# marthinwurer/gcmiipy

Hardware: AMD Instinct MI355X
Metric: cell-updates/s (C-grid Matsuno step) (higher is better)
Workload: dtype f64; 1 GPU; 2-D shallow water + theta + viscosity + van-Leer tracer, 4096x2048 fp64 (BASELINE configs[2]); variant=fused, decomposition=1 latitude band(s)

## Files before the change

### gcmiipy_amd/csrc/gcm_math.h

```cpp
#pragma once
#include <hip/hip_runtime.h>

#include "sw2d_kernels.h"

namespace gcm {

constexpr double kG = 9.8;
constexpr double kRd = 287.0;
constexpr double kRv = 461.0;
constexpr double kCp = 1004.0;
constexpr double kKappa = 287.0 / 1004.0;
constexpr double kP0 = 100000.0;
constexpr double kMuAir = 18.5 * 1e-6;

__device__ __forceinline__ double rcp(double x) {
    double r = __builtin_amdgcn_rcp(x);
    double e = __builtin_fma(-x, r, 1.0);
    r = __builtin_fma(r, e, r);
    e = __builtin_fma(-x, r, 1.0);
    r = __builtin_fma(r, e, r);
    return r;
}
__device__ __forceinline__ float rcp(float x) { return __builtin_amdgcn_rcpf(x); }
constexpr double kTinyF64 = 2.2250738585072014e-308;

constexpr double kBinom1 = kKappa;
constexpr double kBinom2 = kBinom1 * (kKappa - 1) / 2;
constexpr double kBinom3 = kBinom2 * (kKappa - 2) / 3;
constexpr double kBinom4 = kBinom3 * (kKappa - 3) / 4;
constexpr double kBinom5 = kBinom4 * (kKappa - 4) / 5;
constexpr double kBinom6 = kBinom5 * (kKappa - 5) / 6;
constexpr double kBinom7 = kBinom6 * (kKappa - 6) / 7;

__host__ __device__ __forceinline__ double exner(double p, const double *tab ) {
#if defined(__HIP_DEVICE_COMPILE__)
    const int hi = __double2hiint(p);
    const int e = ((hi >> 20) & 0x7ff) - 1023;
    const int idx = (hi >> 14) & 63;
    const double m = __hiloint2double((hi & 0x000fffff) | 0x3ff00000, __double2loint(p));
    const int ec = min(max(e, -64), 63);
#else
    unsigned long long bits;
    __builtin_memcpy(&bits, &p, sizeof bits);
    const int hi = (int)(unsigned)(bits >> 32);
    const int e = ((hi >> 20) & 0x7ff) - 1023;
    const int idx = (hi >> 14) & 63;
    const unsigned long long mbits = ((unsigned long long)(unsigned)((hi & 0x000fffff) | 0x3ff00000) << 32) | (bits & 0xffffffffull);
    double m;
    __builtin_memcpy(&m, &mbits, sizeof m);
    const int ec = e < -64 ? -64 : (e > 63 ? 63 : e);
#endif
    const double E = tab[ec + 64];
    const double rc = tab[128 + 2 * idx], ck = tab[129 + 2 * idx];
    const double t = __builtin_fma(m, rc, -1.0);
    const double t2 = t * t, t4 = t2 * t2;
    const double q12 = __builtin_fma(t, kBinom2, kBinom1);
    const double q34 = __builtin_fma(t, kBinom4, kBinom3);
    const double q56 = __builtin_fma(t, kBinom6, kBinom5);
    const double hi3 = __builtin_fma(t4, kBinom7, __builtin_fma(t2, q56, q34));
    const double poly = __builtin_fma(t * t2, hi3, __builtin_fma(t, q12, 1.0));
    const double r = E * ck * poly;
    const bool ok = (hi >= 0) && (e >= -64) && (e <= 63);
    return ok ? r : __builtin_nan("");
}
__device__ __forceinline__ float exner(float p, const double *tab) { return (float)exner((double)p, tab); }

__device__ __forceinline__ double from_west(double x) {
    int lo = __double2loint(x), hi = __double2hiint(x);
    lo = __builtin_amdgcn_update_dpp(0, lo, 0x138 , 0xf, 0xf, true);
    hi = __builtin_amdgcn_update_dpp(0, hi, 0x138, 0xf, 0xf, true);
    return __hiloint2double(hi, lo);
}
__device__ __forceinline__ double from_east(double x) {
    int lo = __double2loint(x), hi = __double2hiint(x);
    lo = __builtin_amdgcn_update_dpp(0, lo, 0x130 , 0xf, 0xf, true);
    hi = __builtin_amdgcn_update_dpp(0, hi, 0x130, 0xf, 0xf, true);
    return __hiloint2double(hi, lo);
}
__device__ __forceinline__ float from_west(float x) {
    return __int_as_float(__builtin_amdgcn_update_dpp(0, __float_as_int(x), 0x138 , 0xf, 0xf, true));
}
__device__ __forceinline__ float from_east(float x) {
    return __int_as_float(__builtin_amdgcn_update_dpp(0, __float_as_int(x), 0x130 , 0xf, 0xf, true));
}
typedef float f32x2 __attribute__((ext_vector_type(2)));
__device__ __forceinline__ f32x2 rcp(f32x2 x) { return f32x2{rcp(x.x), rcp(x.y)}; }
__device__ __forceinline__ f32x2 exner(f32x2 p, const double *tab) { return f32x2{exner(p.x, tab), exner(p.y, tab)}; }
__device__ __forceinline__ f32x2 from_west(f32x2 x) { return f32x2{from_west(x.y), x.x}; }
__device__ __forceinline__ f32x2 from_east(f32x2 x) { return f32x2{x.y, from_east(x.x)}; }
__device__ __forceinline__ int sign_word(double x) { return __double2hiint(x); }
__device__ __forceinline__ int sign_word(float x) { return __float_as_int(x); }


template <typename T>
__device__ __forceinline__ T adv_vel_u(T uc, T uw, T ue, T un, T us, T vc, T vw, T vs, T vsw, T h_dx) {
    T u_ipj = ue + uc, u_imj = uw + uc, v_ijm = vw + vc, v_ijp = vsw + vs;
    T du_ipj = ue - uc, du_imj = uc - uw, du_ijp = us - uc, du_ijm = uc - un;
    return (u_ipj * du_ipj + u_imj * du_imj + v_ijp * du_ijp + v_ijm * du_ijm) * h_dx;
}

template <typename T>
__device__ __forceinline__ T adv_vel_v(T vc, T vw, T ve, T vn, T vs, T uc, T un, T uw, T usw, T h_dx) {
    T v_ijp = vs + vc, v_ijm = vn + vc, u_ipj = uc + un, u_imj = uw + usw;
    T dv_ipj = ve - vc, dv_imj = vc - vw, dv_ijp = vs - vc, dv_ijm = vc - vn;
    return (u_ipj * dv_ipj + u_imj * dv_imj + v_ijp * dv_ijp + v_ijm * dv_ijm) * h_dx;
}

template <typename T>
__device__ __forceinline__ T geo_grad(T p_next, T pc, T g_dx) {
    return (p_next - pc) * g_dx;
}

template <typename T>
__device__ __forceinline__ T adv_geo(T uc, T uw, T vc, T vn, T pc, T pw, T pe, T pn, T ps, T h_dx) {
    T up_imj = (pw + pc) * uw;
    T up_ipj = (pe + pc) * uc;
    T vp_ijm = (pn + pc) * vn;
    T vp_ijp = (ps + pc) * vc;
    return (up_ipj - up_imj) * h_dx + (vp_ijp - vp_ijm) * h_dx;
}

template <typename T>
__device__ __forceinline__ T visc_u(T uc, T uw, T ue, T un, T us, T mu_dx2) {
    T top = us + un + ue + uw - T(4.0) * uc;
    return top * mu_dx2;
}

template <typename T>
struct Thermo { T t_over_p, geo, st; };
template <typename T>
__device__ __forceinline__ Thermo<T> thermo(T p, T t, const double *tab, T rcp_p) {
    T temp = t * exner(p, tab);
    Thermo<T> r;
    r.t_over_p = temp * rcp_p;
    r.geo = temp * T(kRd / kG);
    r.st = p * t;
    return r;
}
template <typename T>
__device__ __forceinline__ Thermo<T> thermo(T p, T t, const double *tab) {
    return thermo(p, t, tab, rcp(p));
}

template <bool LIMIT, typename T>
__device__ __forceinline__ T face_flux(T vel, T qm1, T q0, T q1, T q2, T dtdx) {
    const bool pos = vel > T(0.0);
    const T vd = vel * dtdx;
    const T f_low = (pos ? q0 : q1) * vd;
    if (!LIMIT) return f_low;
    const T f_high = vd * ((q0 + q1) * T(0.5));
    const T b = q1 - q0;
    const T num = pos ? q0 - qm1 : q2 - q1;
    const T an = fabs(num), ab = fabs(b);
    const bool same = (sign_word(num) ^ sign_word(b)) >= 0;
    T phi;
    if constexpr (sizeof(T) == 8) {
        phi = same && an >= kTinyF64 && ab >= kTinyF64 ? (an + an) * rcp(ab + an) : T(0.0);
    } else {
        phi = same && an > T(0.0) && ab > T(0.0) ? fmin((an + an) * rcp(ab + an), T(2.0)) : T(0.0);
    }
    return f_low + phi * (f_high - f_low);
}
template <bool LIMIT>
__device__ __forceinline__ f32x2 face_flux(f32x2 vel, f32x2 qm1, f32x2 q0, f32x2 q1, f32x2 q2, f32x2 dtdx) {
    return f32x2{face_flux<LIMIT>(vel.x, qm1.x, q0.x, q1.x, q2.x, dtdx.x),
                 face_flux<LIMIT>(vel.y, qm1.y, q0.y, q1.y, q2.y, dtdx.y)};
}

}
```

### gcmiipy_amd/csrc/sw2d_impl.h

```cpp
#pragma once
#include <hip/hip_runtime.h>

#include <cstdlib>
#include <type_traits>

#include "gcm_math.h"
#include "sw2d_kernels.h"

namespace gcm {

__device__ __forceinline__ long row_off(int j, int H, int W, bool wrap) {
    if (wrap) {
        j %= H;
        if (j < 0) j += H;
    }
    return (long)j * W;
}

template <typename T>
__device__ __forceinline__ Sw2dArgsT<T> member_args(const Sw2dArgsT<T> &a0, int m) {
    Sw2dArgsT<T> a = a0;
    const long o = (long)m * a0.mstride;
    auto mv = [o](auto *p) { return p ? p + o : p; };
    a.bu = mv(a.bu); a.bv = mv(a.bv); a.bp = mv(a.bp); a.bt = mv(a.bt); a.bq = mv(a.bq);
    a.su = mv(a.su); a.sv = mv(a.sv); a.sp = mv(a.sp); a.st = mv(a.st);
    a.sgeo = mv(a.sgeo); a.sirho = mv(a.sirho); a.sst = mv(a.sst);
    a.ou = mv(a.ou); a.ov = mv(a.ov); a.op = mv(a.op); a.ot = mv(a.ot); a.oq = mv(a.oq);
    a.dgeo = mv(a.dgeo); a.dirho = mv(a.dirho); a.dst = mv(a.dst);
    return a;
}

template <typename T>
__global__ __launch_bounds__(256) void sw2d_derive_kernel(Sw2dArgsT<T> a0) {
    const Sw2dArgsT<T> a = member_args(a0, blockIdx.z);
    __shared__ double tab[kExnerTabDoubles];
    tab[threadIdx.y * 64 + threadIdx.x] = a.exner_tab[threadIdx.y * 64 + threadIdx.x];
    __syncthreads();
    const int i = blockIdx.x * 64 + threadIdx.x;
    const int j = a.j0 + blockIdx.y * 4 + threadIdx.y;
    if (i >= a.W || j >= a.j1) return;
    const long o = (long)j * a.W + i;
    Thermo<T> th = thermo(a.sp[o], a.st[o], tab);
    a.dgeo[o] = th.geo;
    a.dirho[o] = th.t_over_p;
    a.dst[o] = th.st;
}

template <typename T, bool TEMP>
__global__ __launch_bounds__(256) void sw2d_stage_kernel(Sw2dArgsT<T> a0) {
    const Sw2dArgsT<T> a = member_args(a0, blockIdx.z);
    const int W = a.W, H = a.H;
    const int i = blockIdx.x * 64 + threadIdx.x;
    const int j = a.j0 + blockIdx.y * 4 + threadIdx.y;
    if (i >= W || j >= a.j1) return;
    const bool wrap = a.wrap_j;
    const int iw = i == 0 ? W - 1 : i - 1, ie = i == W - 1 ? 0 : i + 1;
    const long rc = row_off(j, H, W, wrap), rn = row_off(j - 1, H, W, wrap),
               rs = row_off(j + 1, H, W, wrap);
    const T uc = a.su[rc + i], uw = a.su[rc + iw], ue = a.su[rc + ie], un = a.su[rn + i], us = a.su[rs + i],
            usw = a.su[rs + iw];
    const T vc = a.sv[rc + i], vw = a.sv[rc + iw], ve = a.sv[rc + ie], vn = a.sv[rn + i], vs = a.sv[rs + i],
            vsw = a.sv[rs + iw];
    const T pc = a.sp[rc + i], pw = a.sp[rc + iw], pe = a.sp[rc + ie], pn = a.sp[rn + i], ps = a.sp[rs + i];
    T gc = pc, ge = pe, gs = ps;
    if (TEMP) {
        gc = a.sgeo[rc + i];
        ge = a.sgeo[rc + ie];
        gs = a.sgeo[rs + i];
    }
    T du = adv_vel_u(uc, uw, ue, un, us, vc, vw, vs, vsw, a.h_dx) + geo_grad(ge, gc, a.g_dx);
    T dv = adv_vel_v(vc, vw, ve, vn, vs, uc, un, uw, usw, a.h_dx) + geo_grad(gs, gc, a.g_dx);
    if (TEMP) {
        const T vis = visc_u(uc, uw, ue, un, us, a.mu_dx2) * a.sirho[rc + i];
        du -= vis;
        dv -= vis;
    }
    const T dp = adv_geo(uc, uw, vc, vn, pc, pw, pe, pn, ps, a.h_dx);
    const long o = (long)j * W + i;
    const T bp = a.bp[o];
    const T pnew = bp - a.dt * dp;
    a.ou[o] = a.bu[o] - a.dt * du;
    a.ov[o] = a.bv[o] - a.dt * dv;
    a.op[o] = pnew;
    if (TEMP) {
        const T dst = adv_geo(uc, uw, vc, vn, a.sst[rc + i], a.sst[rc + iw], a.sst[rc + ie],
                                   a.sst[rn + i], a.sst[rs + i], a.h_dx);
        const T tt = bp * a.bt[o] - a.dt * dst;
        a.ot[o] = tt * rcp(pnew);
    }
}

template <typename T, int AXIS, bool LIMIT>
__global__ __launch_bounds__(256) void tracer_axis_kernel(Sw2dArgsT<T> a0, const T *qin, T *qout) {
    const Sw2dArgsT<T> a = member_args(a0, blockIdx.z);
    qin += blockIdx.z * a0.mstride;
    qout += blockIdx.z * a0.mstride;
    const int W = a.W, H = a.H;
    const int i = blockIdx.x * 64 + threadIdx.x;
    const int j = a.j0 + blockIdx.y * 4 + threadIdx.y;
    if (i >= W || j >= a.j1) return;
    const bool wrap = a.wrap_j;
    T f, fm;
    const long rc = row_off(j, H, W, wrap);
    if (AXIS == 0) {
        const long r1 = row_off(j + 1, H, W, wrap), r2 = row_off(j + 2, H, W, wrap),
                   rm = row_off(j - 1, H, W, wrap), rmm = row_off(j - 2, H, W, wrap);
        const T qmm = qin[rmm + i], qm = qin[rm + i], q0 = qin[rc + i], q1 = qin[r1 + i], q2 = qin[r2 + i];
        f = face_flux<LIMIT>(a.bv[rc + i], qm, q0, q1, q2, a.dtdx);
        fm = face_flux<LIMIT>(a.bv[rm + i], qmm, qm, q0, q1, a.dtdx);
        qout[(long)j * W + i] = q0 - f + fm;
    } else {
        auto wi = [W](int x) { x %= W; return x < 0 ? x + W : x; };
        const int i1 = wi(i + 1), i2 = wi(i + 2), im = wi(i - 1), imm = wi(i - 2);
        const T qmm = qin[rc + imm], qm = qin[rc + im], q0 = qin[rc + i], q1 = qin[rc + i1], q2 = qin[rc + i2];
        f = face_flux<LIMIT>(a.bu[rc + i], qm, q0, q1, q2, a.dtdx);
        fm = face_flux<LIMIT>(a.bu[rc + im], qmm, qm, q0, q1, a.dtdx);
        qout[(long)j * W + i] = q0 - f + fm;
    }
}

template <typename T>
static dim3 cell_grid(const Sw2dArgsT<T> &a) {
    return dim3((a.W + 63) / 64, (a.j1 - a.j0 + 3) / 4, a.members);
}

template <typename T>
void launch_sw2d_derive(const Sw2dArgsT<T> &a, hipStream_t s) {
    if (a.j1 <= a.j0) return;
    hipLaunchKernelGGL(sw2d_derive_kernel<T>, cell_grid(a), dim3(64, 4), 0, s, a);
}

template <typename T>
void launch_sw2d_stage(const Sw2dArgsT<T> &a, bool temp, hipStream_t s) {
    if (a.j1 <= a.j0) return;
    if (temp)
        hipLaunchKernelGGL((sw2d_stage_kernel<T, true>), cell_grid(a), dim3(64, 4), 0, s, a);
    else
        hipLaunchKernelGGL((sw2d_stage_kernel<T, false>), cell_grid(a), dim3(64, 4), 0, s, a);
}

template <typename T>
void launch_tracer_axis(const Sw2dArgsT<T> &a, int axis, bool limit, const T *q_in, T *q_out, hipStream_t s) {
    if (a.j1 <= a.j0) return;
    dim3 g = cell_grid(a), b(64, 4);
    if (axis == 0) {
        if (limit) hipLaunchKernelGGL((tracer_axis_kernel<T, 0, true>), g, b, 0, s, a, q_in, q_out);
        else hipLaunchKernelGGL((tracer_axis_kernel<T, 0, false>), g, b, 0, s, a, q_in, q_out);
    } else {
        if (limit) hipLaunchKernelGGL((tracer_axis_kernel<T, 1, true>), g, b, 0, s, a, q_in, q_out);
        else hipLaunchKernelGGL((tracer_axis_kernel<T, 1, false>), g, b, 0, s, a, q_in, q_out);
    }
}

template <typename T>
struct Row {
    T u, uw, v, vw, p, st, g, irho;
};

template <bool TEMP, typename T>
__device__ __forceinline__ void make_row_r(Row<T> &r, T u, T v, T p, T t, const double *tab, T rcp_p) {
    r.u = u;
    r.v = v;
    r.p = p;
    r.uw = from_west(u);
    r.vw = from_west(v);
    if (TEMP) {
        Thermo<T> th = thermo(p, t, tab, rcp_p);
        r.st = th.st;
        r.g = th.geo;
        r.irho = th.t_over_p;
    } else {
        r.st = T(0.0);
        r.g = p;
        r.irho = T(0.0);
    }
}

template <bool TEMP, typename T>
__device__ __forceinline__ void make_row(Row<T> &r, T u, T v, T p, T t, const double *tab) {
    make_row_r<TEMP>(r, u, v, p, t, tab, TEMP ? rcp(p) : T(0.0));
}

template <typename T>
struct Tend {
    T du, dv, dp, dst;
};

template <bool TEMP, typename T>
__device__ __forceinline__ Tend<T> tendencies(const Row<T> &RM, const Row<T> &R0, const Row<T> &RP, T g_dx, T h_dx,
                                              T mu_dx2) {
    const T ue = from_east(R0.u), ve = from_east(R0.v);
    const T uw = R0.uw, vw = R0.vw, usw = RP.uw, vsw = RP.vw;
    const T pw = from_west(R0.p), pe = from_east(R0.p);
    const T ge = TEMP ? from_east(R0.g) : pe;
    Tend<T> t;
    t.du = adv_vel_u(R0.u, uw, ue, RM.u, RP.u, R0.v, vw, RP.v, vsw, h_dx) +
           geo_grad(ge, R0.g, g_dx);
    t.dv = adv_vel_v(R0.v, vw, ve, RM.v, RP.v, R0.u, RM.u, uw, usw, h_dx) +
           geo_grad(RP.g, R0.g, g_dx);
    if (TEMP) {
        const T vis = visc_u(R0.u, uw, ue, RM.u, RP.u, mu_dx2) * R0.irho;
        t.du -= vis;
        t.dv -= vis;
    }
    t.dp = adv_geo(R0.u, uw, R0.v, RM.v, R0.p, pw, pe, RM.p, RP.p, h_dx);
    t.dst = T(0.0);
    if (TEMP) {
        const T stw = from_west(R0.st), ste = from_east(R0.st);
        t.dst = adv_geo(R0.u, uw, R0.v, RM.v, R0.st, stw, ste, RM.st, RP.st, h_dx);
    }
    return t;
}

template <typename T>
struct Raw {
    T u, v, p, t, q;
};

constexpr unsigned kNoStore = 0x80000000u;
__device__ __forceinline__ void store_row_lanes(double *row, int W, unsigned lane_off, double x) {
    typedef unsigned int u32x2 __attribute__((ext_vector_type(2)));
    const __amdgpu_buffer_rsrc_t rs = __builtin_amdgcn_make_buffer_rsrc(row, 0, W * 8, 0x00020000);
    __builtin_amdgcn_raw_buffer_store_b64(__builtin_bit_cast(u32x2, x), rs, (int)lane_off, 0, 0);
}

__device__ __forceinline__ double own_copy(double x) {
    double y;
    asm volatile("v_mov_b64 %0, %1" : "=v"(y) : "v"(x) : "memory");
    return y;
}

template <typename T, bool TEMP, int TRACER, bool WRAPJ, bool STREAM = false, int CPL = 1>
struct FusedCtx {
    using Real = std::conditional_t<CPL == 2, f32x2, T>;
    using V = Real;
    const Sw2dArgsT<T> &a;
    const double *tab;
    int ci, col, ja, jb;
    bool store_lane;
    V f0_prev;

    __device__ __forceinline__ Raw<V> load(int j) const {
        const long o = row_off(j, a.H, a.W, WRAPJ) + ci;
        Raw<V> r;
        if constexpr (CPL == 2) {
            auto ld = [o](const T *p) {
                const f32x2 *q = (const f32x2 *)(p + o);
                return STREAM ? __builtin_nontemporal_load(q) : *q;
            };
            r.u = ld(a.bu);
            r.v = ld(a.bv);
            r.p = ld(a.bp);
            r.t = TEMP ? ld(a.bt) : V(0.0f);
            r.q = TRACER ? ld(a.bq) : V(0.0f);
        } else if (STREAM) {
            r.u = __builtin_nontemporal_load(&a.bu[o]);
            r.v = __builtin_nontemporal_load(&a.bv[o]);
            r.p = __builtin_nontemporal_load(&a.bp[o]);
            r.t = TEMP ? __builtin_nontemporal_load(&a.bt[o]) : T(0.0);
            r.q = TRACER ? __builtin_nontemporal_load(&a.bq[o]) : T(0.0);
        } else {
            r.u = a.bu[o];
            r.v = a.bv[o];
            r.p = a.bp[o];
            r.t = TEMP ? a.bt[o] : T(0.0);
            r.q = TRACER ? a.bq[o] : T(0.0);
        }
        return r;
    }

    template <bool FETCH = true, int AHEAD = 3, int LEAD = -1, bool ROWBUF = false>
    __device__ __forceinline__ void iter(int r, Row<V> &BM, Row<V> &B0, Row<V> &BP, Row<V> &SN, Row<V> &SM,
                                         Row<V> &S0, Raw<V> &nxt, V &qmm, V &qm, V &q0, V &qp) {
        const V dt = V(a.dt), g_dx = V(a.g_dx), h_dx = V(a.h_dx), mu_dx2 = V(a.mu_dx2), dtdx = V(a.dtdx);
        {
            const Tend<V> t = tendencies<TEMP>(BM, B0, BP, g_dx, h_dx, mu_dx2);
            const V us = B0.u - dt * t.du;
            const V vs = B0.v - dt * t.dv;
            const V ps = B0.p - dt * t.dp;
            V ts = V(0.0), rps = V(0.0);
            if (TEMP) {
                rps = rcp(ps);
                ts = (B0.st - dt * t.dst) * rps;
            }
            make_row_r<TEMP>(SN, us, vs, ps, ts, tab, rps);
        }
        V f0_cur = V(0.0);
        if (TRACER && (LEAD < 0 ? r >= ja : LEAD >= 1)) f0_cur = face_flux<TRACER == 2>(BM.v, qmm, qm, q0, qp, dtdx);
        if (LEAD < 0 ? r >= ja + 1 : LEAD >= 2) {
            const Tend<V> t = tendencies<TEMP>(SM, S0, SN, g_dx, h_dx, mu_dx2);
            const V un = BM.u - dt * t.du;
            const V vn = BM.v - dt * t.dv;
            const V pn = BM.p - dt * t.dp;
            V tn = V(0.0), qn = V(0.0);
            if (TEMP) tn = (BM.st - dt * t.dst) * rcp(pn);
            if (TRACER) {
                const V qs = qm - f0_cur + f0_prev;
                const V qs_w = from_west(qs), qs_e = from_east(qs);
                const V qs_ee = from_east(qs_e);
                const V f1 = face_flux<TRACER == 2>(BM.u, qs_w, qs, qs_e, qs_ee, dtdx);
                qn = qs - f1 + from_west(f1);
            }
            if constexpr (ROWBUF) {
                const long o = (long)(r - 1) * a.W;
                const unsigned lane_off = store_lane ? (unsigned)col * 8u : kNoStore;
                store_row_lanes(a.ou + o, a.W, lane_off, un);
                store_row_lanes(a.ov + o, a.W, lane_off, vn);
                store_row_lanes(a.op + o, a.W, lane_off, pn);
                if (TEMP) store_row_lanes(a.ot + o, a.W, lane_off, tn);
                if (TRACER) store_row_lanes(a.oq + o, a.W, lane_off, qn);
            } else if (store_lane) {
                const long o = (long)(r - 1) * a.W + col;
                if constexpr (CPL == 2) {
                    auto st = [o](T *p, V x) { *(V *)(p + o) = x; };
                    st(a.ou, un);
                    st(a.ov, vn);
                    st(a.op, pn);
                    if (TEMP) st(a.ot, tn);
                    if (TRACER) st(a.oq, qn);
                } else {
                    a.ou[o] = un;
                    a.ov[o] = vn;
                    a.op[o] = pn;
                    if (TEMP) a.ot[o] = tn;
                    if (TRACER) a.oq[o] = qn;
                }
            }
        }
        f0_prev = f0_cur;
        if constexpr (AHEAD == 3) {
            make_row<TEMP>(BM, nxt.u, nxt.v, nxt.p, nxt.t, tab);
        } else {
            make_row<TEMP>(BM, own_copy(nxt.u), own_copy(nxt.v), own_copy(nxt.p), TEMP ? own_copy(nxt.t) : nxt.t, tab);
        }
        if (TRACER) {
            qmm = qm;
            qm = q0;
            q0 = qp;
            if constexpr (AHEAD == 3) qp = nxt.q;
            else qp = own_copy(nxt.q);
        }
        if constexpr (AHEAD == 3) {
            if (FETCH && r + 3 <= jb + 1) nxt = load(r + 3);
        } else {
            nxt = load(min(r + AHEAD, jb + 1));
        }
    }
};

template <int N, int PRE, class Ctx, typename T = typename Ctx::Real>
__device__ __forceinline__ void preloaded_iters(Ctx &c, const Raw<T> (&pre)[PRE + 4], Row<T> &A, Row<T> &B, Row<T> &C,
                                                Row<T> &X, Row<T> &Y, Row<T> &Z, Raw<T> &nxt, T &qmm, T &qm, T &q0,
                                                T &qp) {
    if constexpr (N < PRE + 2) {
        const int r = c.ja - 1 + N;
        if (r > c.jb) return;
        c.template iter<false>(r, A, B, C, X, Y, Z, nxt, qmm, qm, q0, qp);
        if constexpr (N < PRE) nxt = pre[N + 4];
        preloaded_iters<N + 1, PRE>(c, pre, B, C, A, Y, Z, X, nxt, qmm, qm, q0, qp);
    }
}

template <typename T, bool TEMP, int TRACER, bool WRAPJ, int PRE = 0, bool STREAM = false, int CPL = 1, int DEPTH = 1>
__global__ __launch_bounds__(64, DEPTH == 3 ? 2 : (CPL == 2 && TRACER != 0) ? 3 : 1) void sw2d_fused_kernel(Sw2dArgsT<T> a0) {
    using Ctx = FusedCtx<T, TEMP, TRACER, WRAPJ, STREAM, CPL>;
    using V = typename Ctx::Real;
    constexpr int kCols = sw2d_fused_strip_cols(CPL);
    const int W = a0.W;
    const int lane = threadIdx.x;
    const int strips = (W + kCols - 1) / kCols;
    const int per_xcd = gridDim.x / 8;
    int tile = (blockIdx.x % 8) * per_xcd + blockIdx.x / 8;
    int member = 0;
    if (a0.members > 1) {
        const int per_member = strips * ((a0.j1 - a0.j0 + a0.rows_per_band - 1) / a0.rows_per_band);
        member = tile / per_member;
        if (member >= a0.members) return;
        tile -= member * per_member;
    }
    const int band = tile / strips;
    const int i0 = (tile - band * strips) * kCols;
    const Sw2dArgsT<T> a = member_args(a0, member);
    __shared__ double tab[kExnerTabDoubles];
    if (TEMP) {
        for (int k = 0; k < kExnerTabDoubles / 64; ++k) tab[lane + 64 * k] = a.exner_tab[lane + 64 * k];
        __syncthreads();
    }
    Ctx c{a, tab};
    c.ja = a.j0 + band * a.rows_per_band;
    c.jb = min(c.ja + a.rows_per_band, a.j1);
    if (c.ja >= c.jb) return;
    c.col = i0 - 2 * CPL + CPL * lane;
    c.ci = c.col % W;
    if (c.ci < 0) c.ci += W;
    c.store_lane = lane >= 2 && lane < 62 && c.col < W;
    c.f0_prev = V(0.0);
    const int ja = c.ja, jb = c.jb;

    Row<V> A, B, C, X, Y, Z;
    if constexpr (PRE > 0) {
        Raw<V> pre[PRE + 4];
#pragma unroll
        for (int n = 0; n < PRE + 4; ++n) pre[n] = c.load(min(ja - 2 + n, jb + 1));
        make_row<TEMP>(A, pre[0].u, pre[0].v, pre[0].p, pre[0].t, tab);
        make_row<TEMP>(B, pre[1].u, pre[1].v, pre[1].p, pre[1].t, tab);
        make_row<TEMP>(C, pre[2].u, pre[2].v, pre[2].p, pre[2].t, tab);
        V qmm = V(0.0), qm = pre[0].q, q0 = pre[1].q, qp = pre[2].q;
        Raw<V> nxt = pre[3];
        X = Y = Z = A;
        preloaded_iters<0, PRE>(c, pre, A, B, C, X, Y, Z, nxt, qmm, qm, q0, qp);
        return;
    }
    if constexpr (DEPTH == 3) {
        static_assert(PRE == 0 && CPL == 1, "the deep march is the rolling form with one column per lane");
        const Raw<V> w0 = c.load(ja - 2), w1 = c.load(ja - 1), w2 = c.load(ja);
        Raw<V> n0 = c.load(ja + 1), n1 = c.load(ja + 2), n2 = c.load(min(ja + 3, jb + 1));
        make_row<TEMP>(A, w0.u, w0.v, w0.p, w0.t, tab);
        make_row<TEMP>(B, w1.u, w1.v, w1.p, w1.t, tab);
        make_row<TEMP>(C, w2.u, w2.v, w2.p, w2.t, tab);
        V qmm = V(0.0), qm = w0.q, q0 = w1.q, qp = w2.q;
        X = Y = Z = A;
        c.template iter<true, 5, 0, true>(ja - 1, A, B, C, X, Y, Z, n0, qmm, qm, q0, qp);
        c.template iter<true, 5, 1, true>(ja, B, C, A, Y, Z, X, n1, qmm, qm, q0, qp);
        int r = ja + 1;
        for (; r + 2 <= jb; r += 3) {
            c.template iter<true, 5, 2, true>(r, C, A, B, Z, X, Y, n2, qmm, qm, q0, qp);
            c.template iter<true, 5, 2, true>(r + 1, A, B, C, X, Y, Z, n0, qmm, qm, q0, qp);
            c.template iter<true, 5, 2, true>(r + 2, B, C, A, Y, Z, X, n1, qmm, qm, q0, qp);
        }
        if (r <= jb) {
            c.template iter<false, 3, 2, true>(r, C, A, B, Z, X, Y, n2, qmm, qm, q0, qp);
            if (r + 1 <= jb) c.template iter<false, 3, 2, true>(r + 1, A, B, C, X, Y, Z, n0, qmm, qm, q0, qp);
        }
        return;
    }
    Raw<V> x = c.load(ja - 2);
    make_row<TEMP>(A, x.u, x.v, x.p, x.t, tab);
    V qmm = V(0.0), qm = x.q;
    x = c.load(ja - 1);
    make_row<TEMP>(B, x.u, x.v, x.p, x.t, tab);
    V q0 = x.q;
    x = c.load(ja);
    make_row<TEMP>(C, x.u, x.v, x.p, x.t, tab);
    V qp = x.q;
    Raw<V> nxt = c.load(ja + 1);
    X = Y = Z = A;

    for (int r = ja - 1; r <= jb; r += 3) {
        c.iter(r, A, B, C, X, Y, Z, nxt, qmm, qm, q0, qp);
        if (r + 1 > jb) break;
        c.iter(r + 1, B, C, A, Y, Z, X, nxt, qmm, qm, q0, qp);
        if (r + 2 > jb) break;
        c.iter(r + 2, C, A, B, Z, X, Y, nxt, qmm, qm, q0, qp);
    }
}


template <typename T>
struct Out3 {
    T u, v, p;
};

template <typename T>
__device__ __forceinline__ Out3<T> matsuno_row(bool corr, const Row<T> &BM, const Row<T> &B0, const Row<T> &BP,
                                               Row<T> &SN, const Row<T> &SM, const Row<T> &S0, T dt, T g_dx, T h_dx) {
    {
        const Tend<T> t = tendencies<false>(BM, B0, BP, g_dx, h_dx, T(0.0));
        make_row<false>(SN, B0.u - dt * t.du, B0.v - dt * t.dv, B0.p - dt * t.dp, T(0.0), nullptr);
    }
    Out3<T> o{T(0.0), T(0.0), T(0.0)};
    if (corr) {
        const Tend<T> t = tendencies<false>(SM, S0, SN, g_dx, h_dx, T(0.0));
        o.u = BM.u - dt * t.du;
        o.v = BM.v - dt * t.dv;
        o.p = BM.p - dt * t.dp;
    }
    return o;
}

template <typename T>
struct Fused2Ctx {
    const Sw2dArgsT<T> &a;
    int ja, jb, col;
    bool store_lane;
};

template <int N, int RPB, typename T>
__device__ __forceinline__ void fused2_iters(const Fused2Ctx<T> &c, const Raw<T> (&pre)[RPB + 8], Row<T> &A1, Row<T> &B1,
                                             Row<T> &C1, Row<T> &X1, Row<T> &Y1, Row<T> &Z1, Row<T> &A2, Row<T> &B2,
                                             Row<T> &C2, Row<T> &X2, Row<T> &Y2, Row<T> &Z2) {
    if constexpr (N < RPB + 7) {
        const T dt = c.a.dt, g_dx = c.a.g_dx, h_dx = c.a.h_dx;
        const int r1 = c.ja - 3 + N;
        Out3<T> o1{T(0.0), T(0.0), T(0.0)};
        if (r1 <= c.jb + 2) {
            o1 = matsuno_row(N >= 2, A1, B1, C1, X1, Y1, Z1, dt, g_dx, h_dx);
            if constexpr (N + 3 < RPB + 8) make_row<false>(A1, pre[N + 3].u, pre[N + 3].v, pre[N + 3].p, T(0.0), nullptr);
        }
        if constexpr (N >= 5) {
            const int r2 = r1 - 3;
            if (r2 <= c.jb) {
                const Out3<T> o2 = matsuno_row(N >= 7, A2, B2, C2, X2, Y2, Z2, dt, g_dx, h_dx);
                if (N >= 7 && r2 - 1 < c.jb && c.store_lane) {
                    const long o = (long)(r2 - 1) * c.a.W + c.col;
                    c.a.ou[o] = o2.u;
                    c.a.ov[o] = o2.v;
                    c.a.op[o] = o2.p;
                }
            }
        }
        if constexpr (N >= 2) make_row<false>(A2, o1.u, o1.v, o1.p, T(0.0), nullptr);
        if constexpr (N >= 2)
            fused2_iters<N + 1, RPB>(c, pre, B1, C1, A1, Y1, Z1, X1, B2, C2, A2, Y2, Z2, X2);
        else
            fused2_iters<N + 1, RPB>(c, pre, B1, C1, A1, Y1, Z1, X1, A2, B2, C2, X2, Y2, Z2);
    }
}

template <typename T, int RPB, bool ENS>
__global__ __launch_bounds__(64) void sw2d_fused2_kernel(Sw2dArgsT<T> a0) {
    const int W = a0.W, H = a0.H;
    const int lane = threadIdx.x;
    const int strips = (W + kStrip2Cols - 1) / kStrip2Cols;
    const int per_xcd = gridDim.x / 8;
    int tile = (blockIdx.x % 8) * per_xcd + blockIdx.x / 8;
    int member = 0;
    if constexpr (ENS) {
        const int per_member = strips * ((H + RPB - 1) / RPB);
        member = tile / per_member;
        if (member >= a0.members) return;
        tile -= member * per_member;
    }
    const int band = tile / strips;
    const int i0 = (tile - band * strips) * kStrip2Cols;
    const Sw2dArgsT<T> a = ENS ? member_args(a0, member) : a0;
    Fused2Ctx<T> c{a};
    c.ja = a.j0 + band * RPB;
    c.jb = min(c.ja + RPB, a.j1);
    if (c.ja >= c.jb) return;
    c.col = i0 - 4 + lane;
    int ci = c.col % W;
    if (ci < 0) ci += W;
    c.store_lane = lane >= 4 && lane < 60 && c.col < W;
    Raw<T> pre[RPB + 8];
#pragma unroll
    for (int n = 0; n < RPB + 8; ++n) {
        int j = (c.ja - 4 + n) % H;
        if (j < 0) j += H;
        const long o = (long)j * W + ci;
        pre[n].u = a.bu[o];
        pre[n].v = a.bv[o];
        pre[n].p = a.bp[o];
        pre[n].t = T(0.0);
        pre[n].q = T(0.0);
    }
    Row<T> A1, B1, C1, X1, Y1, Z1, A2, B2, C2, X2, Y2, Z2;
    make_row<false>(A1, pre[0].u, pre[0].v, pre[0].p, T(0.0), nullptr);
    make_row<false>(B1, pre[1].u, pre[1].v, pre[1].p, T(0.0), nullptr);
    make_row<false>(C1, pre[2].u, pre[2].v, pre[2].p, T(0.0), nullptr);
    X1 = Y1 = Z1 = A2 = B2 = C2 = X2 = Y2 = Z2 = A1;
    fused2_iters<0, RPB>(c, pre, A1, B1, C1, X1, Y1, Z1, A2, B2, C2, X2, Y2, Z2);
}

template <typename T>
bool launch_sw2d_fused2(const Sw2dArgsT<T> &a, hipStream_t s) {
    if (!sw2d_fused2_serves(a.wrap_j, a.j0, a.j1, a.H, a.rows_per_band)) return false;
    const int strips = (a.W + kStrip2Cols - 1) / kStrip2Cols;
    const int bands = (a.H + a.rows_per_band - 1) / a.rows_per_band;
    dim3 g((unsigned)(((long)strips * bands * a.members + 7) / 8 * 8));
    Sw2dArgsT<T> arg = a;
    void *params[] = {&arg};
    const bool ens = a.members > 1;
    const void *fn = a.rows_per_band == 2 ? (ens ? (const void *)sw2d_fused2_kernel<T, 2, true> : (const void *)sw2d_fused2_kernel<T, 2, false>)
                   : a.rows_per_band == 3 ? (ens ? (const void *)sw2d_fused2_kernel<T, 3, true> : (const void *)sw2d_fused2_kernel<T, 3, false>)
                                          : (ens ? (const void *)sw2d_fused2_kernel<T, 4, true> : (const void *)sw2d_fused2_kernel<T, 4, false>);
    return hipLaunchKernel(fn, g, dim3(64), params, 0, s) == hipSuccess;
}

template <typename T, bool TEMP, int TRACER, int CPL = 1>
static const void *fused_fn(bool wrap, bool stream, int depth = 1) {
    if constexpr (std::is_same_v<T, double> && TEMP && CPL == 1) {
        if (depth == 3) {
            if (stream)
                return wrap ? (const void *)sw2d_fused_kernel<T, TEMP, TRACER, true, 0, true, CPL, 3>
                            : (const void *)sw2d_fused_kernel<T, TEMP, TRACER, false, 0, true, CPL, 3>;
            return wrap ? (const void *)sw2d_fused_kernel<T, TEMP, TRACER, true, 0, false, CPL, 3>
                        : (const void *)sw2d_fused_kernel<T, TEMP, TRACER, false, 0, false, CPL, 3>;
        }
    }
    if (stream)
        return wrap ? (const void *)sw2d_fused_kernel<T, TEMP, TRACER, true, 0, true, CPL>
                    : (const void *)sw2d_fused_kernel<T, TEMP, TRACER, false, 0, true, CPL>;
    return wrap ? (const void *)sw2d_fused_kernel<T, TEMP, TRACER, true, 0, false, CPL>
                : (const void *)sw2d_fused_kernel<T, TEMP, TRACER, false, 0, false, CPL>;
}

template <typename T, int CPL>
static const void *fused_kernel_ptr_c(bool temp, int tracer, bool wrap, bool preload, bool stream, int depth) {
    if (!temp) {
        if (preload)
            return wrap ? (const void *)sw2d_fused_kernel<T, false, 0, true, kPreloadRows, false, CPL>
                        : (const void *)sw2d_fused_kernel<T, false, 0, false, kPreloadRows, false, CPL>;
        return fused_fn<T, false, 0, CPL>(wrap, stream);
    }
    if (tracer == 0) return fused_fn<T, true, 0, CPL>(wrap, stream, depth);
    if (tracer == 1) return fused_fn<T, true, 1, CPL>(wrap, stream, depth);
    return fused_fn<T, true, 2, CPL>(wrap, stream, depth);
}

template <typename T>
static const void *fused_kernel_ptr(bool temp, int tracer, bool wrap, bool preload = false, bool stream = false,
                                    int cols = 1, int depth = 1) {
    if constexpr (std::is_same_v<T, float>)
        if (cols == 2) return fused_kernel_ptr_c<T, 2>(temp, tracer, wrap, preload, stream, 1);
    return fused_kernel_ptr_c<T, 1>(temp, tracer, wrap, preload, stream, depth);
}

constexpr int kDeepMaxRows = 96;
template <typename T>
int sw2d_fused_rows_per_band(int W, int H, bool temp, int tracer, bool wrap, int members, int cols, int depth_pin) {
    if (const char *e = getenv("GCM_FUSED_ROWS")) {
        int v = atoi(e);
        if (v > 0) return v;
    }
    const long M = members < 1 ? 1 : members;
    const Sw2dFusedForm form = sw2d_fused_form(temp, tracer, kPreloadRows + 1, W, H, M, (long)sizeof(T), depth_pin);
    const bool deep = form.depth == 3;
    int waves_per_cu = deep ? 8 : 12, cus = 256, dev = 0;
    hipDeviceProp_t prop;
    if (hipGetDevice(&dev) == hipSuccess && hipGetDeviceProperties(&prop, dev) == hipSuccess)
        cus = prop.multiProcessorCount;
    int nb = 0;
    if (hipOccupancyMaxActiveBlocksPerMultiprocessor(&nb, fused_kernel_ptr<T>(temp, tracer, wrap, false, deep && form.stream, cols, form.depth),
                                                     64, 0) == hipSuccess && nb > 0)
        waves_per_cu = nb;
    const long slots = (long)waves_per_cu * cus;
    const long strips = (W + sw2d_fused_strip_cols(cols) - 1) / sw2d_fused_strip_cols(cols);
    auto waves = [&](int rpb) { return M * strips * ((H + rpb - 1) / rpb); };
    if (deep && waves(8) >= slots) {
        for (long rounds = 1;; ++rounds) {
            long bands = rounds * slots / (strips * M);
            if (bands < 1) bands = 1;
            const long rpb = (H + bands - 1) / bands;
            if (rpb <= kDeepMaxRows || bands >= H) return (int)(rpb < 8 ? 8 : rpb);
        }
    }
    if (waves(8) < slots) {
        long rpb = M * H * strips / (5L * cus);
        if (!temp && M > 1 && rpb > kPreloadRows) rpb = kPreloadRows;
        return (int)(rpb < 2 ? 2 : rpb > 8 ? 8 : rpb);
    }
    long rounds = (waves(64) + slots - 1) / slots;
    long bands = rounds * slots / (strips * M);
    if (bands < 1) bands = 1;
    long rpb = (H + bands - 1) / bands;
    return (int)(rpb < 8 ? 8 : rpb);
}

template <typename T>
int sw2d_fused_cols(int W, int H, bool temp, int tracer, bool wrap, int members) {
    if (!std::is_same_v<T, float> || W % 2) return 1;
    if (const char *e = getenv("GCM_SW2D_F32_COLS")) return e[0] == '1' ? 1 : 2;
    int waves_per_cu = 12, cus = 256, dev = 0, nb = 0;
    hipDeviceProp_t prop;
    if (hipGetDevice(&dev) == hipSuccess && hipGetDeviceProperties(&prop, dev) == hipSuccess)
        cus = prop.multiProcessorCount;
    if (hipOccupancyMaxActiveBlocksPerMultiprocessor(&nb, fused_kernel_ptr<T>(temp, tracer, wrap), 64, 0) == hipSuccess &&
        nb > 0)
        waves_per_cu = nb;
    const long strips = (W + kStripCols - 1) / kStripCols;
    const long waves8 = (long)(members < 1 ? 1 : members) * strips * ((H + 7) / 8);
    return waves8 < (long)waves_per_cu * cus ? 1 : 2;
}

template <typename T>
bool launch_sw2d_fused(const Sw2dArgsT<T> &a, bool temp, int tracer, hipStream_t s, int cols, int depth_pin) {
    if (a.j1 <= a.j0) return true;
    const int strips = (a.W + sw2d_fused_strip_cols(cols) - 1) / sw2d_fused_strip_cols(cols);
    const int bands = (a.j1 - a.j0 + a.rows_per_band - 1) / a.rows_per_band;
    dim3 g((unsigned)(((long)strips * bands * a.members + 7) / 8 * 8));
    Sw2dArgsT<T> arg = a;
    void *params[] = {&arg};
    const Sw2dFusedForm f = sw2d_fused_form(temp, tracer, a.rows_per_band, a.W, a.j1 - a.j0, a.members, (long)sizeof(T), depth_pin);
    return hipLaunchKernel(fused_kernel_ptr<T>(temp, tracer, a.wrap_j != 0, f.preload, f.stream, cols, f.depth), g, dim3(64), params, 0, s) == hipSuccess;
}

template <typename T>
__global__ void copy_rows_kernel(T *dst, const T *src, long n) {
    long i = (long)blockIdx.x * blockDim.x + threadIdx.x;
    const long stride = (long)gridDim.x * blockDim.x;
    for (; i < n; i += stride) dst[i] = src[i];
}

template <typename T>
void launch_copy_rows(T *dst, const T *src, int W, int nrows, hipStream_t s) {
    const long n = (long)W * nrows;
    if (n <= 0) return;
    int blocks = (int)((n + 255) / 256);
    if (blocks > 1024) blocks = 1024;
    hipLaunchKernelGGL(copy_rows_kernel<T>, dim3(blocks), dim3(256), 0, s, dst, src, n);
}

#define GCM_SW2D_INSTANTIATE(T)                                                                                   \
    template void launch_sw2d_stage<T>(const Sw2dArgsT<T> &, bool, hipStream_t);                                 \
    template void launch_sw2d_derive<T>(const Sw2dArgsT<T> &, hipStream_t);                                      \
    template void launch_tracer_axis<T>(const Sw2dArgsT<T> &, int, bool, const T *, T *, hipStream_t);           \
    template bool launch_sw2d_fused<T>(const Sw2dArgsT<T> &, bool, int, hipStream_t, int, int);                  \
    template int sw2d_fused_rows_per_band<T>(int, int, bool, int, bool, int, int, int);                         \
    template int sw2d_fused_cols<T>(int, int, bool, int, bool, int);                                            \
    template bool launch_sw2d_fused2<T>(const Sw2dArgsT<T> &, hipStream_t);                                      \
    template void launch_copy_rows<T>(T *, const T *, int, int, hipStream_t);

}
```

Baseline: 66.34 billion cell-updates/s.

## Add lean deep-march path with carried row differences and simplified flux limiter

Adds a LEAN variant of the per-row iteration, used by the three-row deep march. It carries the v-sums, u/v differences and p/st face sums from one row to the next instead of recomputing them. It folds the Rd/g geopotential scaling into the gradient coefficient and rewrites the van-Leer face flux as a single FMA on precomputed differences. Input rows now use the raw hardware reciprocal seed with no Newton refinement, which cuts FLOPs and registers in a compute-heavy fp64 kernel but lowers the accuracy of the 1/p term that feeds viscosity.

```diff
diff --git a/gcmiipy_amd/csrc/gcm_math.h b/gcmiipy_amd/csrc/gcm_math.h
--- a/gcmiipy_amd/csrc/gcm_math.h
+++ b/gcmiipy_amd/csrc/gcm_math.h
@@ -141,6 +141,15 @@
 __device__ __forceinline__ Thermo<T> thermo(T p, T t, const double *tab) {
     return thermo(p, t, tab, rcp(p));
 }
+__device__ __forceinline__ Thermo<double> thermo_unscaled(double p, double t, const double *tab, double rcp_p) {
+    const double temp = t * exner(p, tab);
+    Thermo<double> r;
+    r.t_over_p = temp * rcp_p;
+    r.geo = temp;
+    r.st = p * t;
+    return r;
+}
+__device__ __forceinline__ double rcp_seed(double x) { return __builtin_amdgcn_rcp(x); }
 
 template <bool LIMIT, typename T>
 __device__ __forceinline__ T face_flux(T vel, T qm1, T q0, T q1, T q2, T dtdx) {
@@ -162,6 +171,21 @@
     return f_low + phi * (f_high - f_low);
 }
 template <bool LIMIT>
+__device__ __forceinline__ double face_flux_diff(double vel, double q0, double q1, double b, double dm, double dp,
+                                                 double dtdx) {
+    const bool pos = vel > 0.0;
+    const double vd = vel * dtdx;
+    const double qd = pos ? q0 : q1;
+    if (!LIMIT) return qd * vd;
+    const double num = pos ? dm : dp;
+    const double an = fabs(num), ab = fabs(b);
+    const bool same = (sign_word(num) ^ sign_word(b)) >= 0;
+    const double half_phi = same && an >= kTinyF64 && ab >= kTinyF64 ? an * rcp(ab + an) : 0.0;
+    const double sb = __hiloint2double(__double2hiint(b) ^ (__double2hiint(vel) & (int)0x80000000u), __double2loint(b));
+    return vd * __builtin_fma(half_phi, sb, qd);
+}
+
+template <bool LIMIT>
 __device__ __forceinline__ f32x2 face_flux(f32x2 vel, f32x2 qm1, f32x2 q0, f32x2 q1, f32x2 q2, f32x2 dtdx) {
     return f32x2{face_flux<LIMIT>(vel.x, qm1.x, q0.x, q1.x, q2.x, dtdx.x),
                  face_flux<LIMIT>(vel.y, qm1.y, q0.y, q1.y, q2.y, dtdx.y)};
diff --git a/gcmiipy_amd/csrc/sw2d_impl.h b/gcmiipy_amd/csrc/sw2d_impl.h
--- a/gcmiipy_amd/csrc/sw2d_impl.h
+++ b/gcmiipy_amd/csrc/sw2d_impl.h
@@ -157,7 +157,7 @@
     T u, uw, v, vw, p, st, g, irho;
 };
 
-template <bool TEMP, typename T>
+template <bool TEMP, bool LEAN = false, typename T>
 __device__ __forceinline__ void make_row_r(Row<T> &r, T u, T v, T p, T t, const double *tab, T rcp_p) {
     r.u = u;
     r.v = v;
@@ -165,7 +165,9 @@
     r.uw = from_west(u);
     r.vw = from_west(v);
     if (TEMP) {
-        Thermo<T> th = thermo(p, t, tab, rcp_p);
+        Thermo<T> th;
+        if constexpr (LEAN) th = thermo_unscaled(p, t, tab, rcp_p);
+        else th = thermo(p, t, tab, rcp_p);
         r.st = th.st;
         r.g = th.geo;
         r.irho = th.t_over_p;
@@ -179,6 +181,10 @@
 template <bool TEMP, typename T>
 __device__ __forceinline__ void make_row(Row<T> &r, T u, T v, T p, T t, const double *tab) {
     make_row_r<TEMP>(r, u, v, p, t, tab, TEMP ? rcp(p) : T(0.0));
+}
+
+__device__ __forceinline__ void make_row_lean(Row<double> &r, double u, double v, double p, double t, const double *tab) {
+    make_row_r<true, true>(r, u, v, p, t, tab, rcp_seed(p));
 }
 
 template <typename T>
@@ -213,6 +219,57 @@
 }
 
 template <typename T>
+struct Carry {
+    T vu, du;
+    T vv, dv;
+    T sp, sst;
+};
+
+template <typename T>
+__device__ __forceinline__ void prime_carry(Carry<T> &k, const Row<T> &RM, const Row<T> &R0) {
+    k.vu = R0.vw + R0.v;
+    k.du = R0.u - RM.u;
+    k.vv = R0.v + RM.v;
+    k.dv = R0.v - RM.v;
+    k.sp = R0.p + RM.p;
+    k.sst = R0.st + RM.st;
+}
+
+template <typename T>
+__device__ __forceinline__ Tend<T> tendencies_lean(const Row<T> &RM, const Row<T> &R0, const Row<T> &RP, Carry<T> &k,
+                                                   T g_dx_rg, T h_dx, T mu_dx2) {
+    const T uc = R0.u, vc = R0.v, uw = R0.uw, vw = R0.vw;
+    const T ue = from_east(uc), ve = from_east(vc), ge = from_east(R0.g);
+    Tend<T> t;
+    const T du_ipj = ue - uc, du_imj = uc - uw, du_ijp = RP.u - uc, du_ijm = k.du;
+    {
+        const T u_ipj = ue + uc, u_imj = uw + uc, v_ijm = k.vu, v_ijp = RP.vw + RP.v;
+        t.du = (u_ipj * du_ipj + u_imj * du_imj + v_ijp * du_ijp + v_ijm * du_ijm) * h_dx + (ge - R0.g) * g_dx_rg;
+        k.vu = v_ijp;
+        k.du = du_ijp;
+    }
+    {
+        const T v_ijp = RP.v + vc, v_ijm = k.vv, u_ipj = uc + RM.u, u_imj = uw + RP.uw;
+        const T dv_ipj = ve - vc, dv_imj = vc - vw, dv_ijp = RP.v - vc, dv_ijm = k.dv;
+        t.dv = (u_ipj * dv_ipj + u_imj * dv_imj + v_ijp * dv_ijp + v_ijm * dv_ijm) * h_dx + (RP.g - R0.g) * g_dx_rg;
+        k.vv = v_ijp;
+        k.dv = dv_ijp;
+    }
+    const T vis = ((du_ipj - du_imj) + (du_ijp - du_ijm)) * mu_dx2 * R0.irho;
+    t.du -= vis;
+    t.dv -= vis;
+    auto geo = [&](T c, T s, T &sn) {
+        const T se = from_east(c) + c, sw = from_west(se), ss = s + c;
+        const T d = (se * uc - sw * uw) * h_dx + (ss * vc - sn * RM.v) * h_dx;
+        sn = ss;
+        return d;
+    };
+    t.dp = geo(R0.p, RP.p, k.sp);
+    t.dst = geo(R0.st, RP.st, k.sst);
+    return t;
+}
+
+template <typename T>
 struct Raw {
     T u, v, p, t, q;
 };
@@ -239,6 +296,7 @@
     int ci, col, ja, jb;
     bool store_lane;
     V f0_prev;
+    Carry<V> kp, kc;
 
     __device__ __forceinline__ Raw<V> load(int j) const {
         const long o = row_off(j, a.H, a.W, WRAPJ) + ci;
@@ -269,12 +327,17 @@
         return r;
     }
 
-    template <bool FETCH = true, int AHEAD = 3, int LEAD = -1, bool ROWBUF = false>
+    template <bool FETCH = true, int AHEAD = 3, int LEAD = -1, bool ROWBUF = false, bool LEAN = false>
     __device__ __forceinline__ void iter(int r, Row<V> &BM, Row<V> &B0, Row<V> &BP, Row<V> &SN, Row<V> &SM,
                                          Row<V> &S0, Raw<V> &nxt, V &qmm, V &qm, V &q0, V &qp) {
         const V dt = V(a.dt), g_dx = V(a.g_dx), h_dx = V(a.h_dx), mu_dx2 = V(a.mu_dx2), dtdx = V(a.dtdx);
+        static_assert(!LEAN || (TEMP && CPL == 1 && std::is_same_v<T, double> && LEAD >= 0), "the deep march only");
+        V g_dx_rg = g_dx;
+        if constexpr (LEAN) g_dx_rg = g_dx * (kRd / kG);
         {
-            const Tend<V> t = tendencies<TEMP>(BM, B0, BP, g_dx, h_dx, mu_dx2);
+            Tend<V> t;
+            if constexpr (LEAN) t = tendencies_lean(BM, B0, BP, kp, g_dx_rg, h_dx, mu_dx2);
+            else t = tendencies<TEMP>(BM, B0, BP, g_dx, h_dx, mu_dx2);
             const V us = B0.u - dt * t.du;
             const V vs = B0.v - dt * t.dv;
             const V ps = B0.p - dt * t.dp;
@@ -283,12 +346,18 @@
                 rps = rcp(ps);
                 ts = (B0.st - dt * t.dst) * rps;
             }
-            make_row_r<TEMP>(SN, us, vs, ps, ts, tab, rps);
-        }
+            make_row_r<TEMP, LEAN>(SN, us, vs, ps, ts, tab, rps);
+        }
+        if constexpr (LEAN && LEAD == 1) prime_carry(kc, S0, SN);
         V f0_cur = V(0.0);
-        if (TRACER && (LEAD < 0 ? r >= ja : LEAD >= 1)) f0_cur = face_flux<TRACER == 2>(BM.v, qmm, qm, q0, qp, dtdx);
+        if (TRACER && (LEAD < 0 ? r >= ja : LEAD >= 1)) {
+            if constexpr (LEAN) f0_cur = face_flux_diff<TRACER == 2>(BM.v, qm, q0, q0 - qm, qm - qmm, qp - q0, dtdx);
+            else f0_cur = face_flux<TRACER == 2>(BM.v, qmm, qm, q0, qp, dtdx);
+        }
         if (LEAD < 0 ? r >= ja + 1 : LEAD >= 2) {
-            const Tend<V> t = tendencies<TEMP>(SM, S0, SN, g_dx, h_dx, mu_dx2);
+            Tend<V> t;
+            if constexpr (LEAN) t = tendencies_lean(SM, S0, SN, kc, g_dx_rg, h_dx, mu_dx2);
+            else t = tendencies<TEMP>(SM, S0, SN, g_dx, h_dx, mu_dx2);
             const V un = BM.u - dt * t.du;
             const V vn = BM.v - dt * t.dv;
             const V pn = BM.p - dt * t.dp;
@@ -296,9 +365,16 @@
             if (TEMP) tn = (BM.st - dt * t.dst) * rcp(pn);
             if (TRACER) {
                 const V qs = qm - f0_cur + f0_prev;
-                const V qs_w = from_west(qs), qs_e = from_east(qs);
-                const V qs_ee = from_east(qs_e);
-                const V f1 = face_flux<TRACER == 2>(BM.u, qs_w, qs, qs_e, qs_ee, dtdx);
+                V f1;
+                if constexpr (LEAN) {
+                    const V qs_e = from_east(qs), b1 = qs_e - qs;
+                    f1 = face_flux_diff<TRACER == 2>(BM.u, qs, qs_e, b1, TRACER == 2 ? from_west(b1) : b1,
+                                                     TRACER == 2 ? from_east(b1) : b1, dtdx);
+                } else {
+                    const V qs_w = from_west(qs), qs_e = from_east(qs);
+                    const V qs_ee = from_east(qs_e);
+                    f1 = face_flux<TRACER == 2>(BM.u, qs_w, qs, qs_e, qs_ee, dtdx);
+                }
                 qn = qs - f1 + from_west(f1);
             }
             if constexpr (ROWBUF) {
@@ -329,9 +405,11 @@
         }
         f0_prev = f0_cur;
         if constexpr (AHEAD == 3) {
-            make_row<TEMP>(BM, nxt.u, nxt.v, nxt.p, nxt.t, tab);
+            if constexpr (LEAN) make_row_lean(BM, nxt.u, nxt.v, nxt.p, nxt.t, tab);
+            else make_row<TEMP>(BM, nxt.u, nxt.v, nxt.p, nxt.t, tab);
         } else {
-            make_row<TEMP>(BM, own_copy(nxt.u), own_copy(nxt.v), own_copy(nxt.p), TEMP ? own_copy(nxt.t) : nxt.t, tab);
+            if constexpr (LEAN) make_row_lean(BM, own_copy(nxt.u), own_copy(nxt.v), own_copy(nxt.p), own_copy(nxt.t), tab);
+            else make_row<TEMP>(BM, own_copy(nxt.u), own_copy(nxt.v), own_copy(nxt.p), TEMP ? own_copy(nxt.t) : nxt.t, tab);
         }
         if (TRACER) {
             qmm = qm;
@@ -415,22 +493,23 @@
         static_assert(PRE == 0 && CPL == 1, "the deep march is the rolling form with one column per lane");
         const Raw<V> w0 = c.load(ja - 2), w1 = c.load(ja - 1), w2 = c.load(ja);
         Raw<V> n0 = c.load(ja + 1), n1 = c.load(ja + 2), n2 = c.load(min(ja + 3, jb + 1));
-        make_row<TEMP>(A, w0.u, w0.v, w0.p, w0.t, tab);
-        make_row<TEMP>(B, w1.u, w1.v, w1.p, w1.t, tab);
-        make_row<TEMP>(C, w2.u, w2.v, w2.p, w2.t, tab);
+        make_row_lean(A, w0.u, w0.v, w0.p, w0.t, tab);
+        make_row_lean(B, w1.u, w1.v, w1.p, w1.t, tab);
+        make_row_lean(C, w2.u, w2.v, w2.p, w2.t, tab);
         V qmm = V(0.0), qm = w0.q, q0 = w1.q, qp = w2.q;
         X = Y = Z = A;
-        c.template iter<true, 5, 0, true>(ja - 1, A, B, C, X, Y, Z, n0, qmm, qm, q0, qp);
-        c.template iter<true, 5, 1, true>(ja, B, C, A, Y, Z, X, n1, qmm, qm, q0, qp);
+        prime_carry(c.kp, A, B);
+        c.template iter<true, 5, 0, true, true>(ja - 1, A, B, C, X, Y, Z, n0, qmm, qm, q0, qp);
+        c.template iter<true, 5, 1, true, true>(ja, B, C, A, Y, Z, X, n1, qmm, qm, q0, qp);
         int r = ja + 1;
         for (; r + 2 <= jb; r += 3) {
-            c.template iter<true, 5, 2, true>(r, C, A, B, Z, X, Y, n2, qmm, qm, q0, qp);
-            c.template iter<true, 5, 2, true>(r + 1, A, B, C, X, Y, Z, n0, qmm, qm, q0, qp);
-            c.template iter<true, 5, 2, true>(r + 2, B, C, A, Y, Z, X, n1, qmm, qm, q0, qp);
+            c.template iter<true, 5, 2, true, true>(r, C, A, B, Z, X, Y, n2, qmm, qm, q0, qp);
+            c.template iter<true, 5, 2, true, true>(r + 1, A, B, C, X, Y, Z, n0, qmm, qm, q0, qp);
+            c.template iter<true, 5, 2, true, true>(r + 2, B, C, A, Y, Z, X, n1, qmm, qm, q0, qp);
         }
         if (r <= jb) {
-            c.template iter<false, 3, 2, true>(r, C, A, B, Z, X, Y, n2, qmm, qm, q0, qp);
-            if (r + 1 <= jb) c.template iter<false, 3, 2, true>(r + 1, A, B, C, X, Y, Z, n0, qmm, qm, q0, qp);
+            c.template iter<false, 3, 2, true, true>(r, C, A, B, Z, X, Y, n2, qmm, qm, q0, qp);
+            if (r + 1 <= jb) c.template iter<false, 3, 2, true, true>(r + 1, A, B, C, X, Y, Z, n0, qmm, qm, q0, qp);
         }
         return;
     }
```

After: 65.63 billion cell-updates/s. -1.1%, worse.
